# cscott/compressjs

Hardware: AMD Instinct MI355X
Metric: bzip2 -9 compress MB/s on enwik8-shaped input (higher is better)
Workload: dtype u8; 1 GPU; synthetic enwik8-shaped text with phrase reuse calibrated to enwik8's bzip2 -9 ratio (compressjs_amd.synth.enwik_like, seed 2025), 100000000 bytes per GPU, bzip2 -9, 899981-byte blocks; BASELINE.json configs[2]; input_bytes=100000000, compressed_bytes=29488912, blocks_in_flight=128

## Files before the change

### compressjs_amd/csrc/cjs_abi.hip

```cpp
#include "../../include/compressjs_amd.h"
#include "cjs_common.h"
#include "k1_bwt.h"
#include "pipeline.h"
#include "bwtc_host.h"
#include "decode_host.h"
#include <vector>
#include <atomic>
#include <chrono>
#include <thread>
#include <functional>
#include <mutex>
#include <condition_variable>
#include <string.h>
#include <stdlib.h>

static int ensure_device() {
    int n = 0;
    if (hipGetDeviceCount(&n) != hipSuccess || n <= 0) return CJS_E_NOGPU;
    return CJS_OK;
}

static int32_t bwt_batch_impl(const uint8_t* T, const uint32_t* nlen, uint32_t nb, uint32_t cap,
                              uint8_t* U, uint32_t* pidx, int reps, float* ms_out, int linear = 0,
                              int32_t* SAout = nullptr) {
// ... 89 lines not shown
    if (n == 0) return CJS_OK;
    if (!SA) return CJS_E_ARG;
    std::vector<u8> u(n);
    u32 p = 0;
    return bwt_batch_impl(T, &n, 1, n, u.data(), &p, 0, nullptr, 1, SA);
}

extern "C" int32_t cjs_unbwt_linear(const uint8_t* T, uint8_t* U, uint32_t n, uint32_t pidx) {
    if (n == 0) return CJS_OK;
    if (!T || !U || pidx > n) return CJS_E_ARG;
    int rc = ensure_device();
    if (rc) return rc;
    u8 *dT = nullptr, *dU = nullptr; void* ws = nullptr;
    hipStream_t st = nullptr;
    hipError_t e;
    const size_t wsb = (size_t)n * 20 + ((size_t)(n + 4095) / 4096) * 1024 + 256;
#define TRY(x) if ((e = (x)) != hipSuccess) { rc = CJS_E_HIP - (int)e; goto done; }
    TRY(hipStreamCreate(&st));
    TRY(hipMalloc((void**)&dT, n));
    TRY(hipMalloc((void**)&dU, n));
    TRY(hipMalloc(&ws, wsb));
    TRY(hipMemcpyAsync(dT, T, n, hipMemcpyHostToDevice, st));
    TRY(hipMemsetAsync(dU, 0, n, st));
    rc = k6_unbwt_linear(dT, dU, n, pidx, ws, st);
    if (rc) goto done;
    TRY(hipStreamSynchronize(st));
    TRY(hipMemcpy(U, dU, n, hipMemcpyDeviceToHost));
done:
    if (st) (void)hipStreamDestroy(st);
    (void)hipFree(dT); (void)hipFree(dU); (void)hipFree(ws);
    return rc;
#undef TRY
}

extern "C" int32_t cjs_huff_lengths_batch(int64_t* arr, const uint32_t* off, uint32_t count, uint32_t max_len) {
    if (count == 0) return CJS_OK;
    if (!arr || !off || max_len < 1 || max_len > 62) return CJS_E_ARG;
    for (u32 k = 0; k < count; k++) {
        if (off[k + 1] < off[k]) return CJS_E_ARG;
        const u64 len = off[k + 1] - off[k];
        if (len > (1ull << max_len)) return CJS_E_ARG;
    }
    const u32 total = off[count];
    if (total == 0) return CJS_OK;
    int rc = ensure_device();
    if (rc) return rc;
    long long* d_arr = nullptr; u32* d_off = nullptr;
    hipError_t e;
#define TRY(x) if ((e = (x)) != hipSuccess) { rc = CJS_E_HIP - (int)e; goto done; }
    TRY(hipMalloc((void**)&d_arr, (size_t)total * 8));
    TRY(hipMalloc((void**)&d_off, (size_t)(count + 1) * 4));
    TRY(hipMemcpy(d_arr, arr, (size_t)total * 8, hipMemcpyHostToDevice));
    TRY(hipMemcpy(d_off, off, (size_t)(count + 1) * 4, hipMemcpyHostToDevice));
    rc = k3_alloc_lengths_run(d_arr, d_off, count, (int)max_len, nullptr);
    if (rc) goto done;
    TRY(hipDeviceSynchronize());
    TRY(hipMemcpy(arr, d_arr, (size_t)total * 8, hipMemcpyDeviceToHost));
done:
    (void)hipFree(d_arr); (void)hipFree(d_off);
    return rc;
#undef TRY
}
extern "C" int32_t cjs_huff_lengths(int64_t* arr, uint32_t n, uint32_t max_len) {
    const uint32_t off[2] = {0, n};
    return cjs_huff_lengths_batch(arr, off, 1, max_len);
}

extern "C" int32_t cjs_bwt_cyclic(const uint8_t* T, uint8_t* U, uint32_t n, uint32_t* pidx) {
    if (n == 0) { if (pidx) *pidx = 0; return CJS_OK; }
    return cjs_bwt_cyclic_batch(T, &n, 1, n, U, pidx);
}

extern "C" int32_t cjs_dbg_block_stages(const uint8_t* T, const uint32_t* nlen, uint32_t nb, uint32_t cap,
                                        int upto, cjs_dbg_stage_out* o) {
    void* dout = nullptr;
    if (!T || !nlen || !o || nb == 0 || cap == 0 || cap > (1u << 22) - 1) return CJS_E_ARG;
    int rc = ensure_device();
    if (rc) return rc;
    BatchGeom g = make_geom(nb, cap);
    u32 max_n = 0;
    std::vector<u8> text((size_t)nb * g.tstride, 0);
    for (u32 b = 0; b < nb; b++) {
        const u32 n = nlen[b];
        if (n > cap || n == 0) return CJS_E_ARG;
        if (n > max_n) max_n = n;
        u8* dst = text.data() + (size_t)b * g.tstride;
        memcpy(dst, T + (size_t)b * cap, n);
        for (u32 i = 0; i < K1_TPAD; i++) dst[n + i] = dst[i % n];
    }
    void* ws = nullptr;
    hipStream_t st = nullptr;
    hipError_t e;
    Pipe P;
#define TRY(x) if ((e = (x)) != hipSuccess) { rc = CJS_E_HIP - (int)e; goto done; }
    TRY(hipStreamCreate(&st));
    TRY(hipMalloc(&ws, pipe_bytes(g)));
    pipe_carve(P, g, ws);
    TRY(hipMemcpyAsync(P.T, text.data(), text.size(), hipMemcpyHostToDevice, st));
    TRY(hipMemcpyAsync(P.nlen, nlen, nb * 4, hipMemcpyHostToDevice, st));
    TRY(hipMemsetAsync(P.pidx, 0, nb * 4, st));
    if (o->crc_in) { TRY(hipMemcpyAsync(P.crc, o->crc_in, nb * 4, hipMemcpyHostToDevice, st)); }
    else { TRY(hipMemsetAsync(P.crc, 0, nb * 4, st)); }
    if (upto >= 5) {
        P.outCapBytes = ((size_t)nb * ((size_t)cap * 2 + 8192) + 4096 + 255) & ~(size_t)255;
        TRY(hipMalloc(&dout, P.outCapBytes));
        P.out = (u32*)dout;
        rc = k5_stream_begin(P, o->level ? o->level : 9, st);
        if (rc) goto done;
    }
    rc = pipe_run_block_stages(P, max_n, st, upto);
    if (rc) goto done;
    if (upto >= 5) { rc = k5_stream_end(P, st); if (rc) goto done; }
    TRY(hipStreamSynchronize(st));
#define BACK2D(dst, src, rowbytes, srcpitch, dstpitch)                                            \
    if (dst) for (u32 b = 0; b < nb; b++)                                                        \
        TRY(hipMemcpy((char*)(dst) + (size_t)b * (dstpitch), (const char*)(src) + (size_t)b * (srcpitch), \
                      (rowbytes), hipMemcpyDeviceToHost));
    BACK2D(o->U, P.U, max_n, g.stride, cap);
    BACK2D(o->pidx, P.pidx, 4, 4, 4);
    if (upto >= 2) {
        BACK2D(o->A, P.A, ((size_t)max_n + 1) * 2, (size_t)g.stride * 2, ((size_t)cap + 1) * 2);
        BACK2D(o->pos, P.pos, 4, 4, 4);
        BACK2D(o->alpha, P.alpha, 4, 4, 4);
        BACK2D(o->freq, P.freq, 258 * 4, K2_FREQ_PITCH * 4, 258 * 4);
        BACK2D(o->used, P.used, 32, 32, 32);
    }
    if (upto >= 3) {
        BACK2D(o->sel, P.sel, (max_n + 1) / 50 + 2, P.selPitch, (cap + 1) / 50 + 2);
        for (int t = 0; t < 6; t++) {
            BACK2D(o->lens ? o->lens + t * 258 : nullptr, P.lens + t * CJS_LEN_PITCH, 258,
                   CJS_MAX_GROUPS * CJS_LEN_PITCH, 6 * 258);
        }
        BACK2D(o->ngroups, P.ngroups, 4, 4, 4);
        BACK2D(o->nsel, P.nsel, 4, 4, 4);
    }
    if (upto >= 5) {
        BACK2D(o->bitlen, P.bitlen, 8, 8, 8);
        StreamState hs;
        TRY(hipMemcpy(&hs, P.ss, sizeof hs, hipMemcpyDeviceToHost));
        if (hs.overflow) { rc = CJS_E_NOSPACE; goto done; }
        o->stream_bytes = (hs.bits + 7) >> 3;
        if (o->stream && o->stream_cap >= o->stream_bytes) {
            TRY(hipMemcpy(o->stream, P.out, o->stream_bytes, hipMemcpyDeviceToHost));
        }
    }
done:
    if (st) (void)hipStreamDestroy(st);
    (void)hipFree(ws);
    (void)hipFree(dout);
    return rc;
#undef TRY
#undef BACK2D
}

#define CJS_PIN_WORDS 8192u
#define CJS_NSTREAMS 4

struct BwtcBlockJob { u32 len, pidx, nsym, ntri; u32 used[8]; size_t off; bool host; size_t soff; };
struct PinnedU32 {
    u32* p = nullptr; size_t cap = 0;
    int reserve(size_t n) {
        if (n <= cap) return CJS_OK;
        if (p) (void)hipHostFree(p);
        p = nullptr; cap = 0;
        n += n / 8 + 1024;
        const hipError_t e = hipHostMalloc((void**)&p, n * sizeof(u32), hipHostMallocDefault);
        if (e != hipSuccess) { p = nullptr; return CJS_E_HIP - (int)e; }
        cap = n;
        return CJS_OK;
    }
    u32* data() { return p; }
    ~PinnedU32() { if (p) (void)hipHostFree(p); }
// ... 1626 lines not shown
```

### compressjs_amd/csrc/k34_huff.hip

```cpp
#include "pipeline.h"
#include <atomic>

#define HB_PITCH 264
#ifdef K34_TRACE
#define K34_NOW() wall_clock64()
#else
#define K34_NOW() 0ll
#endif
static_assert(HB_PITCH == CJS_LEN_PITCH, "fr2's rows (pipeline.hip) have the pitch of the LDS rows");

template <typename I>
__device__ __forceinline__ int ha_mod(I x, int len) {
    return x < (I)len ? (int)x : x < (I)(2 * len) ? (int)x - len : (int)(x % len);
}

template <typename I>
__device__ int ha_first(const I* a, int len, int i, int nodes_to_move) {
    const int limit = i;
    int k = len - 2;
    while (i >= nodes_to_move && ha_mod(a[i], len) > limit) { k = i; i -= (limit - i + 1); }
    if (i < nodes_to_move - 1) i = nodes_to_move - 1;
    while (k > i + 1) {
        const int t = (i + k) >> 1;
        if (ha_mod(a[t], len) > limit) k = t; else i = t;
    }
    return k;
}

template <typename I>
__device__ void ha_parents(I* a, int len) {
    a[0] += a[1];
    {
        const I none = (I)(~(unsigned long long)0 >> (65 - 8 * sizeof(I)));
        int head = 0, top = 2;
        I vh = a[0];
        I vt = top < len ? a[top] : none;
        for (int tail = 1; tail < len - 1; tail++) {
            I t;
            if (top >= len || vh < vt) { t = vh; a[head++] = tail; vh = head < tail ? a[head] : none; }
            else { t = vt; top++; vt = top < len ? a[top] : none; }
            if (top >= len || (head < tail && vh < vt)) { t += vh; a[head++] = tail + len; vh = head < tail ? a[head] : none; }
            else { t += vt; top++; vt = top < len ? a[top] : none; }
            a[tail] = t;
            if (head == tail) vh = t;
        }
    }
}

template <typename I>
__device__ void ha_depths_serial(I* a, int len, int maxlen) {
    int reloc = len - 2;
    for (int d = 1; d < maxlen - 1 && reloc > 1; d++) reloc = ha_first(a, len, reloc - 1, 0);
    if (ha_mod(a[0], len) >= reloc) {
        int first = len - 2, next = len - 1;
        for (int depth = 1, avail = 2; avail > 0; depth++) {
            const int last = first;
            first = ha_first(a, len, last - 1, 0);
            for (int i = avail - (last - first); i > 0; i--) a[next--] = depth;
            avail = (last - first) << 1;
        }
    } else {
        const int nodes_to_move = reloc;
        int fl = 0;
        for (u32 v = (u32)(reloc - 1); v; v >>= 1) fl++;
        const int insert_depth = maxlen - fl;
        int first = len - 2, next = len - 1;
        int depth = (insert_depth == 1) ? 2 : 1;
        int left = (insert_depth == 1) ? nodes_to_move - 2 : nodes_to_move;
        for (int avail = depth << 1; avail > 0; depth++) {
            const int last = first;
            first = (first <= nodes_to_move) ? first : ha_first(a, len, last - 1, nodes_to_move);
            int offset = 0;
            if (depth >= insert_depth) {
                const int capv = 1 << (depth - insert_depth);
                offset = left < capv ? left : capv;
            } else if (depth == insert_depth - 1) {
                offset = 1;
                if (a[first] == last) first++;
            }
            for (int i = avail - (last - first + offset); i > 0; i--) a[next--] = depth;
            left -= offset;
            avail = (last - first + offset) << 1;
        }
    }
// ... 53 lines not shown
            const int last = first;
            if (first > ntm) {
                int below = 0;
                for (int k0 = 0; k0 < root; k0 += 64) {
                    const int k = k0 + lane;
                    below += (int)__popcll(__ballot(k < root && ha_mod(a[k], len) < last));
                }
                first = below > ntm ? below : ntm;
            }
            int offset = 0;
            if (depth >= insert_depth) {
                const int capv = 1 << (depth - insert_depth);
                offset = left < capv ? left : capv;
            } else if (depth == insert_depth - 1) {
                offset = 1;
                if (a[first] == (I)last) first++;
            }
            const int fill = avail - (last - first + offset);
            if (lane == 0 && fill > 0) cnt[64 + depth] = fill;
            left -= offset;
            avail = (last - first + offset) << 1;
        }
        __builtin_amdgcn_wave_barrier();
        const int f = cnt[64 + lane];
        const int cum = (int)wave_incl_scan_u32((u32)f);
        __builtin_amdgcn_wave_barrier();
        cnt[64 + lane] = cum;
        deep = depth - 2;
    } else {
        const int above = __shfl_up(c, 1);
        const int nl = lane >= 1 ? 2 * above - c : 0;
        cnt[64 + lane] = (int)wave_incl_scan_u32((u32)nl);
    }
    __builtin_amdgcn_wave_barrier();
    for (int j = lane; j < len; j += 64) {
        const int r = len - j;
        int dep = 1;
        for (int D = 1; D <= deep; D++) dep += cnt[64 + D] < r ? 1 : 0;
        a[j] = (I)dep;
    }
    __builtin_amdgcn_wave_barrier();
    return true;
}

__device__ void huff_build_wave(const u32* freq, int S, u8* lens, int* keys, int* arr, int* anc, int* dist, int* cnt, u32* tr = nullptr) {
    const int lane = (int)(threadIdx.x & 63u);
    long long t0_ = tr ? K34_NOW() : 0;
    for (int i = lane; i < S; i += 64) keys[i] = (int)((freq[i] << 9) | (u32)i);
    __builtin_amdgcn_wave_barrier();
    {
        constexpr int M = (CJS_MAX_SYMS + 63) / 64;
        int k[M], r[M];
#pragma unroll
        for (int m = 0; m < M; m++) { const int i = lane + 64 * m; k[m] = i < S ? keys[i] : 0; r[m] = 0; }
        for (int j = 0; j < S; j++) {
            const int kj = keys[j];
#pragma unroll
            for (int m = 0; m < M; m++) r[m] += kj < k[m] ? 1 : 0;
        }
#pragma unroll
        for (int m = 0; m < M; m++) if (lane + 64 * m < S) arr[r[m]] = k[m];
    }
    __builtin_amdgcn_wave_barrier();
    for (int i = lane; i < S; i += 64) keys[i] = arr[i];
    __builtin_amdgcn_wave_barrier();
    for (int i = lane; i < S; i += 64) arr[i] = (int)((u32)keys[i] >> 9);
    __builtin_amdgcn_wave_barrier();
    if (tr && lane == 0) { const long long t1_ = K34_NOW(); atomicAdd(tr, (u32)(t1_ - t0_)); t0_ = t1_; }
    if (lane == 0) ha_parents(arr, S);
    __builtin_amdgcn_wave_barrier();
    if (tr && lane == 0) { const long long t1_ = K34_NOW(); atomicAdd(tr + 1, (u32)(t1_ - t0_)); t0_ = t1_; }
    if (!ha_depths_wave(arr, S, CJS_MAX_BITS, anc, dist, cnt)) {
        if (lane == 0) ha_depths_serial(arr, S, CJS_MAX_BITS);
    }
    if (tr && lane == 0) atomicAdd(tr + 2, (u32)(K34_NOW() - t0_));
    __builtin_amdgcn_wave_barrier();
    for (int i = lane; i < S; i += 64) lens[keys[i] & 0x1FF] = (u8)arr[i];
    __builtin_amdgcn_wave_barrier();
}

#define K34_STAGE_WORDS 1600
#define K34_GROUPS_PER_CHUNK 64
#define K34_PRE ((K34_STAGE_WORDS + 63) / 64)

template <class Body, class Done>
__device__ __forceinline__ void walk_groups(const u16* A, u32 pos, u32 nSel, u32* stage_w, u32 c0, u32 cstep, Body body, Done done) {
    const u32 lane = threadIdx.x & 63u;
    const u32* Aw = (const u32*)A;
    const u32 nchunks = (nSel + K34_GROUPS_PER_CHUNK - 1) / K34_GROUPS_PER_CHUNK;
    u32 pre[K34_PRE];
    auto fetch = [&](u32 c) {
        const u32 sym0 = c * K34_GROUPS_PER_CHUNK * CJS_GROUP;
        const u32 nsym = pos - sym0 < 2u * K34_STAGE_WORDS ? pos - sym0 : 2u * K34_STAGE_WORDS;
        const u32 nwords = (nsym + 1u) >> 1;
#pragma unroll
        for (int k = 0; k < K34_PRE; k++) {
            const u32 j = lane + 64u * (u32)k;
            pre[k] = j < nwords ? Aw[(sym0 >> 1) + j] : 0u;
        }
    };
    if (c0 < nchunks) fetch(c0);
    for (u32 c = c0; c < nchunks; c += cstep) {
        const u32 g0 = c * K34_GROUPS_PER_CHUNK;
#pragma unroll
        for (int k = 0; k < K34_PRE; k++) {
            const u32 j = lane + 64u * (u32)k;
            if (j < K34_STAGE_WORDS) stage_w[j] = pre[k];
        }
        __builtin_amdgcn_wave_barrier();
        if (c + cstep < nchunks) fetch(c + cstep);
        const u32 gi = g0 + lane;
        if (lane < K34_GROUPS_PER_CHUNK && gi < nSel) {
            const u32 cnt = pos - gi * CJS_GROUP < CJS_GROUP ? pos - gi * CJS_GROUP : CJS_GROUP;
            const u32* gw = stage_w + lane * 25u;
            if (cnt == CJS_GROUP) {
                u32 wd[CJS_GROUP / 2];
#pragma unroll
                for (int k = 0; k < CJS_GROUP / 2; k++) wd[k] = gw[k];
#pragma unroll
                for (int k = 0; k < CJS_GROUP / 2; k++) { body(gi, wd[k] & 0xFFFFu); body(gi, wd[k] >> 16); }
            } else {
                for (u32 k = 0; k < cnt; k += 2) {
                    const u32 wd = gw[k >> 1];
                    body(gi, wd & 0xFFFFu);
                    if (k + 1 < cnt) body(gi, wd >> 16);
                }
            }
            done(gi);
        }
        __builtin_amdgcn_wave_barrier();
    }
}

#ifndef K34_SPLIT
#define K34_SPLIT 2
#endif
#define K34_MAX_SEL 18432
#ifdef K34_TRACE
#define K34_T0 long long tprev_ = wall_clock64();
#define K34_STAMP(slot) do { __syncthreads(); if (blockIdx.x == 0 && threadIdx.x == 0) { const long long now_ = wall_clock64(); atomicAdd(&P.k1.stats[K1_STAT_RTRACE + (slot)], (u32)(now_ - tprev_)); tprev_ = now_; } } while (0)
#else
#define K34_T0
#define K34_STAMP(slot) do { } while (0)
#endif

struct K34Blk {
    u32 pos, nSel;
    int S, target;
};
__device__ __forceinline__ K34Blk k34_blk(const Pipe& P, u32 b) {
    K34Blk k;
    k.pos = P.pos[b];
    k.S = (int)P.alpha[b] + 2;
    k.nSel = (k.pos + CJS_GROUP - 1) / CJS_GROUP;
    k.target = k.pos >= 2400 ? 6 : k.pos >= 1200 ? 5 : k.pos >= 600 ? 4 : k.pos >= 200 ? 3 : 2;
    return k;
}

__global__ __launch_bounds__(1024) void k34_assign(Pipe P, u32 it) {
    const BatchGeom g = P.g;
    const u32 b = blockIdx.x / K34_SPLIT, k = blockIdx.x % K34_SPLIT;
    if (P.nlen[b] == 0) return;
    const K34Blk q = k34_blk(P, b);
    const int G = 2 + (int)it, S = q.S;
    if (G > q.target) return;
    const u32 tid = threadIdx.x, w = tid >> 6, lane = tid & 63u;
    const u16* A = P.A + (size_t)b * g.stride;
    u8* sel = P.sel + (size_t)b * P.selPitch;
    u16* cost = P.selCost + (size_t)b * P.selPitch;

    HIP_DYNAMIC_SHARED(u32, pool)
    __shared__ u8 lens[CJS_MAX_GROUPS][HB_PITCH];
    __shared__ u32 fr[CJS_MAX_GROUPS][HB_PITCH];
    __shared__ u64 lens64[HB_PITCH];
    u32* stage_w = pool + w * K34_STAGE_WORDS;
    int (*keys)[HB_PITCH] = (int (*)[HB_PITCH])pool;
    int (*arr)[HB_PITCH] = (int (*)[HB_PITCH])(pool + CJS_MAX_GROUPS * HB_PITCH);
    int (*anc)[HB_PITCH] = (int (*)[HB_PITCH])(pool + 2 * CJS_MAX_GROUPS * HB_PITCH);
    int (*dst)[HB_PITCH] = (int (*)[HB_PITCH])(pool + 3 * CJS_MAX_GROUPS * HB_PITCH);
    int (*dcn)[128] = (int (*)[128])(pool + 4 * CJS_MAX_GROUPS * HB_PITCH);

    u32* rows = P.fr2 + ((size_t)b * 2 + (it & 1u)) * CJS_MAX_GROUPS * HB_PITCH;
    u32* next = P.fr2 + ((size_t)b * 2 + ((it + 1u) & 1u)) * CJS_MAX_GROUPS * HB_PITCH;
    K34_T0
    if (it == 0) {
        const u32* gfreq = P.freq + (size_t)b * K2_FREQ_PITCH;
        for (u32 i = tid; i < (u32)S; i += 1024) { fr[0][i] = gfreq[i]; fr[1][i] = 1; }
    } else {
        for (u32 i = tid; i < (u32)G * HB_PITCH; i += 1024) (&fr[0][0])[i] = rows[i];
    }
    if (k == 0 && G < q.target)
        for (u32 i = tid; i < (u32)(CJS_MAX_GROUPS * HB_PITCH); i += 1024) next[i] = 0;
    __syncthreads();
    K34_STAMP(0);
#ifdef K34_TRACE
    if (w < (u32)G) huff_build_wave(fr[w], S, lens[w], keys[w], arr[w], anc[w], dst[w], dcn[w], blockIdx.x == 0 && w == 0 ? P.k1.stats + K1_STAT_RTRACE + 7 : nullptr);
#else
    if (w < (u32)G) huff_build_wave(fr[w], S, lens[w], keys[w], arr[w], anc[w], dst[w], dcn[w]);
#endif
    __syncthreads();
    K34_STAMP(1);
    for (u32 i = tid; i < (u32)S; i += 1024) {
        u64 v = 0;
        for (int t = 0; t < G; t++) v |= (u64)lens[t][i] << (10 * t);
        lens64[i] = v;
    }
    __syncthreads();
    {
        u64 acc = 0;
        walk_groups(A, q.pos, q.nSel, stage_w, k * 16u + w, 16u * K34_SPLIT,
            [&](u32, u32 sym) { acc += lens64[sym]; },
            [&](u32 gi) {
                u32 best = 0, bc = (u32)(acc & 1023u);
                for (int t = 1; t < G; t++) {
                    const u32 c = (u32)((acc >> (10 * t)) & 1023u);
                    if (c < bc) { best = (u32)t; bc = c; }
                }
                sel[gi] = (u8)best;
                cost[gi] = (u16)bc;
                acc = 0;
            });
    }
    K34_STAMP(2);
    if (G < q.target || k != 0) return;
    if (w < (u32)G) {
        const int l = (int)lane;
        const bool mine = l >= 1 && l <= CJS_MAX_BITS;
        u32 count = 0;
        if (mine) for (int i = 0; i < S; i++) count += lens[w][i] == l ? 1u : 0u;
        u32 c = 0, first = 0; int prev = 0;
        for (int ll = 1; ll <= CJS_MAX_BITS; ll++) {
            const u32 cl = (u32)__shfl((int)count, ll);
            if (!cl) continue;
            c <<= (ll - prev);
            if (ll == l) first = c;
            c += cl;
            prev = ll;
        }
        u32* codes = P.codes + ((size_t)b * CJS_MAX_GROUPS + w) * CJS_LEN_PITCH;
        u8* lout = P.lens + ((size_t)b * CJS_MAX_GROUPS + w) * CJS_LEN_PITCH;
        if (mine && count) for (int i = 0; i < S; i++) if (lens[w][i] == l) codes[i] = first++;
        for (int i = l; i < S; i += 64) lout[i] = lens[w][i];
    }
    if (tid == 0) { P.ngroups[b] = (u32)G; P.nsel[b] = q.nSel; }
    K34_STAMP(3);
}

__global__ __launch_bounds__(1024) void k34_split(Pipe P, u32 it) {
    const BatchGeom g = P.g;
    const u32 b = blockIdx.x / K34_SPLIT, k = blockIdx.x % K34_SPLIT;
    if (P.nlen[b] == 0) return;
    const K34Blk q = k34_blk(P, b);
    const int G = 2 + (int)it;
    if (G >= q.target) return;
    const u32 tid = threadIdx.x, w = tid >> 6;
    const u32 nSel = q.nSel;
    const u16* A = P.A + (size_t)b * g.stride;
    const u8* sel = P.sel + (size_t)b * P.selPitch;
    const u16* cost = P.selCost + (size_t)b * P.selPitch;

    HIP_DYNAMIC_SHARED(u32, pool)
    __shared__ u32 fr[CJS_MAX_GROUPS][HB_PITCH];
    __shared__ u32 chist[1024];
    __shared__ u32 cnt[8];
    __shared__ u32 scan_sh[20];
    __shared__ u32 s_which, s_cstar, s_keep;
    __shared__ __attribute__((aligned(16))) u8 selL[K34_MAX_SEL];
    u32* stage_w = pool + w * K34_STAGE_WORDS;
    K34_T0
    u16* costL = (u16*)pool;
    for (u32 i = tid; i < (nSel + 3u) >> 2; i += 1024) ((u32*)selL)[i] = ((const u32*)sel)[i];
    for (u32 i = tid; i < (nSel + 1u) >> 1; i += 1024) ((u32*)costL)[i] = ((const u32*)cost)[i];
    if (tid < 8) cnt[tid] = 0;
    chist[tid] = 0;
    for (u32 i = tid; i < (u32)(CJS_MAX_GROUPS * HB_PITCH); i += 1024) (&fr[0][0])[i] = 0;
    __syncthreads();
    for (u32 g0 = 0; g0 < nSel; g0 += 1024) {
        const u32 gi = g0 + tid;
        const u32 v = gi < nSel ? selL[gi] : 0xFFu;
        for (int t = 0; t < G; t++) {
            const u64 m = __ballot(v == (u32)t);
            if ((tid & 63u) == 0 && m) atomicAdd(&cnt[t], (u32)__popcll(m));
        }
    }
    __syncthreads();
    if (tid == 0) {
        u32 wh = 0;
        for (int t = 1; t < G; t++) if (cnt[t] > cnt[wh]) wh = (u32)t;
        s_which = wh;
    }
    __syncthreads();
    const u32 which = s_which;
    for (u32 gi = tid; gi < nSel; gi += 1024)
        if (selL[gi] == which) atomicAdd(&chist[costL[gi]], 1u);
    __syncthreads();
    {
        const u32 half = cnt[which] >> 1;
        u32 tot;
        const u32 mine = chist[tid];
        const u32 lower = block_excl_scan_1024(mine, scan_sh, &tot);
        if (lower <= half && half < lower + mine) { s_cstar = tid; s_keep = half - lower; }
    }
    __syncthreads();
    {
        const u32 cstar = s_cstar, keep = s_keep;
        const u32 chunk = (nSel + 1023u) / 1024u;
        const u32 lo = tid * chunk < nSel ? tid * chunk : nSel;
        const u32 hi = lo + chunk < nSel ? lo + chunk : nSel;
        u32 eq = 0;
        for (u32 gi = lo; gi < hi; gi++) eq += (selL[gi] == which && costL[gi] == cstar) ? 1u : 0u;
        u32 total;
        u32 rank = block_excl_scan_1024(eq, scan_sh, &total);
        for (u32 gi = lo; gi < hi; gi++) {
            u32 v = selL[gi];
            if (v == which) {
                const u32 c = costL[gi];
                if (c > cstar) v = (u32)G;
                else if (c == cstar) { if (rank >= keep) v = (u32)G; rank++; }
            }
            selL[gi] = (u8)v;
        }
    }
    __syncthreads();
    K34_STAMP(4);
    {
        u64 hot = 0;
        walk_groups(A, q.pos, nSel, stage_w, k * 16u + w, 16u * K34_SPLIT,
            [&](u32 gi, u32 sym) {
                if (sym < 8u) hot += 1ull << (8u * sym);
                else atomicAdd(&fr[selL[gi]][sym], 1u);
            },
            [&](u32 gi) {
                u32* row = fr[selL[gi]];
#pragma unroll
                for (u32 sy = 0; sy < 8u; sy++) {
                    const u32 c = (u32)(hot >> (8u * sy)) & 255u;
                    if (c) atomicAdd(&row[sy], c);
                }
                hot = 0;
            });
    }
    __syncthreads();
    K34_STAMP(5);
    u32* next = P.fr2 + ((size_t)b * 2 + ((it + 1u) & 1u)) * CJS_MAX_GROUPS * HB_PITCH;
    for (u32 i = tid; i < (u32)(CJS_MAX_GROUPS * HB_PITCH); i += 1024) {
        const u32 v = (&fr[0][0])[i];
        if (v) atomicAdd(&next[i], v);
    }
    K34_STAMP(6);
}

int k34_run(Pipe P, hipStream_t stream) {
    const size_t dyn = (size_t)16 * K34_STAGE_WORDS * 4;
    static std::atomic<unsigned> lds_set[64];
    int dev = 0;
    HIP_CHECK_RET(hipGetDevice(&dev));
    if (dev < 0 || dev >= 64 || !lds_set[dev].load(std::memory_order_acquire)) {
        HIP_CHECK_RET(hipFuncSetAttribute((const void*)k34_assign, hipFuncAttributeMaxDynamicSharedMemorySize, (int)(16 * K34_STAGE_WORDS * 4)));
        HIP_CHECK_RET(hipFuncSetAttribute((const void*)k34_split, hipFuncAttributeMaxDynamicSharedMemorySize, (int)(16 * K34_STAGE_WORDS * 4)));
        if (dev >= 0 && dev < 64) lds_set[dev].store(1u, std::memory_order_release);
    }
    if (P.selPitch > K34_MAX_SEL) return CJS_E_ARG;
    for (u32 it = 0; it + 2u <= CJS_MAX_GROUPS; it++) {
        hipLaunchKernelGGL(k34_assign, dim3(P.g.nb * K34_SPLIT), dim3(1024), dyn, stream, P, it);
        if (it + 3u <= CJS_MAX_GROUPS) hipLaunchKernelGGL(k34_split, dim3(P.g.nb * K34_SPLIT), dim3(1024), dyn, stream, P, it);
    }
    HIP_CHECK_RET(hipGetLastError());
#ifdef K34_TRACE
    {
        u32 h[10];
        HIP_CHECK_RET(hipMemcpyAsync(h, P.k1.stats + K1_STAT_RTRACE, sizeof h, hipMemcpyDeviceToHost, stream));
        HIP_CHECK_RET(hipStreamSynchronize(stream));
        fprintf(stderr, "k34 trace (us, block 0 / workgroup 0, summed over iterations): assign load %.1f build %.1f lens64+walk %.1f codes %.1f | split count/median/move %.1f recount %.1f flush %.1f | table 0: sort %.1f parents %.1f depths %.1f\n",
                h[0] / 100.0, h[1] / 100.0, h[2] / 100.0, h[3] / 100.0, h[4] / 100.0, h[5] / 100.0, h[6] / 100.0, h[7] / 100.0, h[8] / 100.0, h[9] / 100.0);
    }
#endif
    return CJS_OK;
}

#define K3_WAVE_MAX 2048
__global__ __launch_bounds__(64) void k3_alloc_lengths(long long* arr, const u32* off, u32 count, int maxlen) {
    const u32 t = blockIdx.x;
    if (t >= count) return;
    __shared__ int anc[K3_WAVE_MAX], dist[K3_WAVE_MAX], cnt[128];
    long long* a = arr + off[t];
    const int len = (int)(off[t + 1] - off[t]);
    const bool one = threadIdx.x == 0;
    if (len == 2) { if (one) { a[0] = 1; a[1] = 1; } }
    else if (len == 1) { if (one) a[0] = 1; }
    else if (len > K3_WAVE_MAX || maxlen > HA_DCAP - 1) { if (one) ha_allocate<long long>(a, len, maxlen); }
    else if (len > 2) {
        if (one) ha_parents<long long>(a, len);
        __syncthreads();
        if (!ha_depths_wave<long long>(a, len, maxlen, anc, dist, cnt)) {
            if (one) ha_depths_serial<long long>(a, len, maxlen);
        }
    }
}
int k3_alloc_lengths_run(long long* d_arr, const u32* d_off, u32 count, int maxlen, hipStream_t stream) {
    hipLaunchKernelGGL(k3_alloc_lengths, dim3(count), dim3(64), 0, stream, d_arr, d_off, count, maxlen);
    HIP_CHECK_RET(hipGetLastError());
    return CJS_OK;
}
```

### compressjs_amd/csrc/pipeline.h

```cpp
#pragma once
#include "cjs_common.h"
#include "devutil.h"
#include "k1_bwt.h"

#define K2_SEG 1024
#define K2_FREQ_PITCH 260
#define CJS_MAX_SYMS 258
#define CJS_MAX_GROUPS 6
#define CJS_GROUP 50
#define CJS_MAX_BITS 20
#define CJS_LEN_PITCH 264

#define K5_NONE (-0x40000000)
#define K5_TGROUPS 80u
#define K5_TILE (K5_TGROUPS * CJS_GROUP)
#define K5_TILES(g) ((g).stride / K5_TILE + 2u)
#define K5_HDR_WORDS 6144

struct StreamState {
    u64 bits;
    u32 crc;
    u32 overflow;
};

struct Pipe {
    BatchGeom g;
    u32 segs;
    u8* T;
    u32* nlen;
    u32* crc;
    K1Buf k1;
    u8* U;
    u32* pidx;
    u32* used;
    u32* alpha;
    u32* nruns;
    u32* tileCnt;
    u32* symCnt;
    u8* RHsym;
    u32* RHpos;
    int* Ltab;
    u8* J;
    u16* A;
    u32* pos;
    u32* freq;
    u8* sel;
    u32 selPitch;
    u8* lens;
    u32* codes;
    u32* ngroups;
    u32* nsel;
    u16* selCost;
    u32* fr2;
    u32* hdr;
    u32* hbits;
    u32* tileBits;
    u64* bitlen;
    u64* bitoff;
    StreamState* ss;
    u32* out;
    u64 outCapBytes;
    u64* snap;
};

struct K0Buf {
    const u8* in;
    u64 in_len;
    u64 ntiles;
    u64 nchunks;
    u32 maxBlocks;
    u64* tileA;
    u64* tileB;
    u64* tileC;
    u64* chunk;
    u64* blkStart;
    u64* blkEnd;
    u64* blkAdj;
    u64* blkRe;
    u32* blkN;
    u32* nBlocks;
    u64* specEnd;
    u64* specC;
    u64* specBad;
};
size_t k0_bytes(u64 in_len, u32 cap);
void k0_carve(K0Buf& K, const u8* d_in, u64 in_len, u32 cap, void* ws);
int k0_prepass(K0Buf K, u32 cap, hipStream_t stream);
#define K0_PHASE_FAIL 0xFFFFFFFFu
int k0_scans(K0Buf K, hipStream_t stream);
int k0_eval(K0Buf K, u64 pos, hipStream_t stream);
int k0_phase_plan(K0Buf K, u32 cap, u64 t0, u64 own_len, u32 last, u64 total, hipStream_t stream);

int k6_unbwt_linear(const u8* dT, u8* dU, u32 n, u32 pidx, void* ws, hipStream_t stream);
int k2_run(Pipe P, u32 max_n, hipStream_t stream);
int k10_model_run(Pipe P, u32* sylt, u32* tot, u32* ntri, u32 ostride, u32 ocap, hipStream_t stream);
int k34_run(Pipe P, hipStream_t stream);
int k3_alloc_lengths_run(long long* d_arr, const u32* d_off, u32 count, int maxlen, hipStream_t stream);
int k5_run(Pipe P, u32 max_n, hipStream_t stream, hipEvent_t after = nullptr, hipEvent_t done = nullptr, hipEvent_t crc_ready = nullptr);
int k5_stream_begin(Pipe P, int level, hipStream_t stream, bool zero = true);
int k5_stream_end(Pipe P, hipStream_t stream);
int k5_shift_bits_run(const u8* d_in, u64 nbytes, u32 s, u8* d_out, hipStream_t stream);
int k0_batch(K0Buf K, Pipe P, u32 first_block, u32 cap, hipStream_t stream, u32 crc_parts, hipStream_t side = nullptr, hipEvent_t ev_pad = nullptr, hipEvent_t ev_crc = nullptr);
size_t pipe_bytes(const BatchGeom& g);
void pipe_carve(Pipe& P, const BatchGeom& g, void* base);
int pipe_run_block_stages(Pipe& P, u32 max_n, hipStream_t stream, int upto, hipEvent_t after = nullptr,
                          hipEvent_t done = nullptr);
```

### compressjs_amd/csrc/pipeline.hip

```cpp
#include "pipeline.h"
#include <string.h>

static inline size_t al256(size_t x) { return (x + 255) & ~(size_t)255; }

size_t pipe_bytes(const BatchGeom& g) {
    size_t tot = 0;
    tot += al256((size_t)g.nb * g.tstride);
    tot += al256((size_t)g.nb * g.stride);
    tot += al256((size_t)g.nb * (g.stride + 1) * 4);
    tot += 2 * al256((size_t)g.nb * g.stride);
    tot += al256((size_t)g.nb * (g.stride / K2_SEG) * 256 * 4);
    tot += al256((size_t)g.nb * g.stride * 2);
    tot += 2 * al256((size_t)g.nb * g.rtiles * 4);
    tot += 16 * al256((size_t)g.nb * 8 * 4);
    tot += al256((size_t)g.nb * K2_FREQ_PITCH * 4);
    const u32 selPitch = (g.stride / CJS_GROUP + 64) & ~63u;
    tot += al256((size_t)g.nb * selPitch);
    tot += al256((size_t)g.nb * CJS_MAX_GROUPS * CJS_LEN_PITCH);
    tot += al256((size_t)g.nb * CJS_MAX_GROUPS * CJS_LEN_PITCH * 4);
    tot += al256((size_t)g.nb * selPitch * 2);
    tot += al256((size_t)g.nb * 2 * CJS_MAX_GROUPS * CJS_LEN_PITCH * 4);
    tot += al256((size_t)g.nb * K5_HDR_WORDS * 4);
    tot += al256((size_t)g.nb * K5_TILES(g) * 4);
    tot += 4 * al256((size_t)g.nb * 8);
    tot += k1_workspace_bytes(g);
    return tot;
}

void pipe_carve(Pipe& P, const BatchGeom& g, void* base) {
    memset(&P, 0, sizeof P);
    P.g = g;
    P.segs = g.stride / K2_SEG;
    char* p = (char*)base;
#define TAKE(field, type, bytes) P.field = (type)p; p += al256(bytes)
    TAKE(T, u8*, (size_t)g.nb * g.tstride);
    TAKE(U, u8*, (size_t)g.nb * g.stride);
    TAKE(RHpos, u32*, (size_t)g.nb * (g.stride + 1) * 4);
    TAKE(RHsym, u8*, (size_t)g.nb * g.stride);
    TAKE(J, u8*, (size_t)g.nb * g.stride);
    TAKE(Ltab, int*, (size_t)g.nb * P.segs * 256 * 4);
    TAKE(A, u16*, (size_t)g.nb * g.stride * 2);
    TAKE(tileCnt, u32*, (size_t)g.nb * g.rtiles * 4);
    TAKE(symCnt, u32*, (size_t)g.nb * g.rtiles * 4);
    TAKE(nlen, u32*, (size_t)g.nb * 4);
    TAKE(crc, u32*, (size_t)g.nb * 4);
    TAKE(pidx, u32*, (size_t)g.nb * 4);
    TAKE(used, u32*, (size_t)g.nb * 8 * 4);
    TAKE(alpha, u32*, (size_t)g.nb * 4);
    TAKE(nruns, u32*, (size_t)g.nb * 4);
    TAKE(pos, u32*, (size_t)g.nb * 4);
    TAKE(ngroups, u32*, (size_t)g.nb * 4);
    TAKE(nsel, u32*, (size_t)g.nb * 4);
    TAKE(bitlen, u64*, (size_t)g.nb * 8);
    TAKE(bitoff, u64*, (size_t)(g.nb + 1) * 8);
    TAKE(freq, u32*, (size_t)g.nb * K2_FREQ_PITCH * 4);
    P.selPitch = (g.stride / CJS_GROUP + 64) & ~63u;
    TAKE(sel, u8*, (size_t)g.nb * P.selPitch);
    TAKE(lens, u8*, (size_t)g.nb * CJS_MAX_GROUPS * CJS_LEN_PITCH);
    TAKE(codes, u32*, (size_t)g.nb * CJS_MAX_GROUPS * CJS_LEN_PITCH * 4);
    TAKE(selCost, u16*, (size_t)g.nb * P.selPitch * 2);
    TAKE(fr2, u32*, (size_t)g.nb * 2 * CJS_MAX_GROUPS * CJS_LEN_PITCH * 4);
    TAKE(hdr, u32*, (size_t)g.nb * K5_HDR_WORDS * 4);
    TAKE(tileBits, u32*, (size_t)g.nb * K5_TILES(g) * 4);
    TAKE(hbits, u32*, (size_t)g.nb * 4);
    TAKE(ss, StreamState*, sizeof(StreamState));
#undef TAKE
    p = (char*)(((uintptr_t)p + 255) & ~(uintptr_t)255);
    k1_carve(P.k1, g, p);
    P.k1.T = P.T;
    P.k1.nlen = P.nlen;
    P.k1.U = P.U;
    P.k1.pidx = P.pidx;
}

int pipe_run_block_stages(Pipe& P, u32 max_n, hipStream_t stream, int upto, hipEvent_t after, hipEvent_t done) {
    int rc = k1_run(P.k1, P.g, max_n, stream);
    if (rc || upto <= 1) return rc;
    rc = k2_run(P, max_n, stream);
    if (rc || upto <= 2) return rc;
    rc = k34_run(P, stream);
    if (rc || upto <= 4) return rc;
    return k5_run(P, max_n, stream, after, done);
}
```

Before: 15700 MB/s.

## Split k34 table refinement into tables/cost/median/recount kernels with wide grids

Restructures each Huffman-table refinement iteration from two per-block 1024-thread kernels (two workgroups per block) into four kernels. Table building runs once per block and writes lens64 to global memory. The group-cost walk and the frequency recount run as 2D grids with many small 256-thread workgroups per block, and per-table group counts are accumulated atomically during the cost pass, so the median kernel no longer needs its own counting pass. The aim is to spread the group walks across far more CUs than before and drop the dynamic-LDS setup; in exchange it adds kernel launches, global round-trips for lens64 and sel, and more global atomics. It also lets the debug-stage entry point skip zero-length blocks instead of rejecting them.

```diff
diff --git a/compressjs_amd/csrc/cjs_abi.hip b/compressjs_amd/csrc/cjs_abi.hip
--- a/compressjs_amd/csrc/cjs_abi.hip
+++ b/compressjs_amd/csrc/cjs_abi.hip
@@ -195,12 +195,14 @@
     std::vector<u8> text((size_t)nb * g.tstride, 0);
     for (u32 b = 0; b < nb; b++) {
         const u32 n = nlen[b];
-        if (n > cap || n == 0) return CJS_E_ARG;
+        if (n > cap) return CJS_E_ARG;
+        if (n == 0) continue;
         if (n > max_n) max_n = n;
         u8* dst = text.data() + (size_t)b * g.tstride;
         memcpy(dst, T + (size_t)b * cap, n);
         for (u32 i = 0; i < K1_TPAD; i++) dst[n + i] = dst[i % n];
     }
+    if (max_n == 0) return CJS_E_ARG;
     void* ws = nullptr;
     hipStream_t st = nullptr;
     hipError_t e;
diff --git a/compressjs_amd/csrc/k34_huff.hip b/compressjs_amd/csrc/k34_huff.hip
--- a/compressjs_amd/csrc/k34_huff.hip
+++ b/compressjs_amd/csrc/k34_huff.hip
@@ -1,5 +1,4 @@
 #include "pipeline.h"
-#include <atomic>
 
 #define HB_PITCH 264
 #ifdef K34_TRACE
@@ -219,12 +218,19 @@
 #define K34_STAGE_WORDS 1600
 #define K34_GROUPS_PER_CHUNK 64
 #define K34_PRE ((K34_STAGE_WORDS + 63) / 64)
-
-template <class Body, class Done>
-__device__ __forceinline__ void walk_groups(const u16* A, u32 pos, u32 nSel, u32* stage_w, u32 c0, u32 cstep, Body body, Done done) {
+#define K34_WALK_WAVES 4
+#ifndef K34_CPW
+#define K34_CPW 4
+#endif
+#define K34_WG_CHUNKS (K34_WALK_WAVES * K34_CPW)
+static_assert(K34_GROUPS_PER_CHUNK * K34_CPW < 1024, "k34_cost sums a wave's per-table group counts in 10-bit fields");
+
+template <class Begin, class Body, class Done>
+__device__ __forceinline__ void walk_groups(const u16* A, u32 pos, u32 nSel, u32* stage_w, u32 c0, u32 cstep, u32 cend, Begin begin, Body body, Done done) {
     const u32 lane = threadIdx.x & 63u;
     const u32* Aw = (const u32*)A;
-    const u32 nchunks = (nSel + K34_GROUPS_PER_CHUNK - 1) / K34_GROUPS_PER_CHUNK;
+    const u32 nall = (nSel + K34_GROUPS_PER_CHUNK - 1) / K34_GROUPS_PER_CHUNK;
+    const u32 nchunks = nall < cend ? nall : cend;
     u32 pre[K34_PRE];
     auto fetch = [&](u32 c) {
         const u32 sym0 = c * K34_GROUPS_PER_CHUNK * CJS_GROUP;
@@ -250,6 +256,7 @@
         if (lane < K34_GROUPS_PER_CHUNK && gi < nSel) {
             const u32 cnt = pos - gi * CJS_GROUP < CJS_GROUP ? pos - gi * CJS_GROUP : CJS_GROUP;
             const u32* gw = stage_w + lane * 25u;
+            begin(gi);
             if (cnt == CJS_GROUP) {
                 u32 wd[CJS_GROUP / 2];
 #pragma unroll
@@ -269,15 +276,12 @@
     }
 }
 
-#ifndef K34_SPLIT
-#define K34_SPLIT 2
-#endif
 #define K34_MAX_SEL 18432
 #ifdef K34_TRACE
-#define K34_T0 long long tprev_ = wall_clock64();
-#define K34_STAMP(slot) do { __syncthreads(); if (blockIdx.x == 0 && threadIdx.x == 0) { const long long now_ = wall_clock64(); atomicAdd(&P.k1.stats[K1_STAT_RTRACE + (slot)], (u32)(now_ - tprev_)); tprev_ = now_; } } while (0)
+#define K34_T0(pred) const bool traced_ = (pred); long long tprev_ = wall_clock64();
+#define K34_STAMP(slot) do { __syncthreads(); if (traced_ && threadIdx.x == 0) { const long long now_ = wall_clock64(); atomicAdd(&P.k1.stats[K1_STAT_RTRACE + (slot)], (u32)(now_ - tprev_)); tprev_ = now_; } } while (0)
 #else
-#define K34_T0
+#define K34_T0(pred)
 #define K34_STAMP(slot) do { } while (0)
 #endif
 
@@ -294,72 +298,50 @@
     return k;
 }
 
-__global__ __launch_bounds__(1024) void k34_assign(Pipe P, u32 it) {
-    const BatchGeom g = P.g;
-    const u32 b = blockIdx.x / K34_SPLIT, k = blockIdx.x % K34_SPLIT;
+__global__ __launch_bounds__(512) void k34_tables(Pipe P, u32 it) {
+    const u32 b = blockIdx.x;
     if (P.nlen[b] == 0) return;
     const K34Blk q = k34_blk(P, b);
     const int G = 2 + (int)it, S = q.S;
     if (G > q.target) return;
     const u32 tid = threadIdx.x, w = tid >> 6, lane = tid & 63u;
-    const u16* A = P.A + (size_t)b * g.stride;
-    u8* sel = P.sel + (size_t)b * P.selPitch;
-    u16* cost = P.selCost + (size_t)b * P.selPitch;
-
-    HIP_DYNAMIC_SHARED(u32, pool)
+
     __shared__ u8 lens[CJS_MAX_GROUPS][HB_PITCH];
     __shared__ u32 fr[CJS_MAX_GROUPS][HB_PITCH];
-    __shared__ u64 lens64[HB_PITCH];
-    u32* stage_w = pool + w * K34_STAGE_WORDS;
-    int (*keys)[HB_PITCH] = (int (*)[HB_PITCH])pool;
-    int (*arr)[HB_PITCH] = (int (*)[HB_PITCH])(pool + CJS_MAX_GROUPS * HB_PITCH);
-    int (*anc)[HB_PITCH] = (int (*)[HB_PITCH])(pool + 2 * CJS_MAX_GROUPS * HB_PITCH);
-    int (*dst)[HB_PITCH] = (int (*)[HB_PITCH])(pool + 3 * CJS_MAX_GROUPS * HB_PITCH);
-    int (*dcn)[128] = (int (*)[128])(pool + 4 * CJS_MAX_GROUPS * HB_PITCH);
+    __shared__ int keys[CJS_MAX_GROUPS][HB_PITCH], arr[CJS_MAX_GROUPS][HB_PITCH];
+    __shared__ int anc[CJS_MAX_GROUPS][HB_PITCH], dst[CJS_MAX_GROUPS][HB_PITCH];
+    __shared__ int dcn[CJS_MAX_GROUPS][128];
 
     u32* rows = P.fr2 + ((size_t)b * 2 + (it & 1u)) * CJS_MAX_GROUPS * HB_PITCH;
     u32* next = P.fr2 + ((size_t)b * 2 + ((it + 1u) & 1u)) * CJS_MAX_GROUPS * HB_PITCH;
-    K34_T0
+    K34_T0(b == 0)
     if (it == 0) {
         const u32* gfreq = P.freq + (size_t)b * K2_FREQ_PITCH;
-        for (u32 i = tid; i < (u32)S; i += 1024) { fr[0][i] = gfreq[i]; fr[1][i] = 1; }
+        for (u32 i = tid; i < (u32)S; i += 512) { fr[0][i] = gfreq[i]; fr[1][i] = 1; }
     } else {
-        for (u32 i = tid; i < (u32)G * HB_PITCH; i += 1024) (&fr[0][0])[i] = rows[i];
-    }
-    if (k == 0 && G < q.target)
-        for (u32 i = tid; i < (u32)(CJS_MAX_GROUPS * HB_PITCH); i += 1024) next[i] = 0;
+        for (u32 i = tid; i < (u32)G * HB_PITCH; i += 512) (&fr[0][0])[i] = rows[i];
+    }
+    if (G < q.target) {
+        for (u32 i = tid; i < (u32)(CJS_MAX_GROUPS * HB_PITCH); i += 512) next[i] = 0;
+        if (tid < 8) P.tabCnt[(size_t)b * 8 + tid] = 0;
+    }
     __syncthreads();
     K34_STAMP(0);
 #ifdef K34_TRACE
-    if (w < (u32)G) huff_build_wave(fr[w], S, lens[w], keys[w], arr[w], anc[w], dst[w], dcn[w], blockIdx.x == 0 && w == 0 ? P.k1.stats + K1_STAT_RTRACE + 7 : nullptr);
+    if (w < (u32)G) huff_build_wave(fr[w], S, lens[w], keys[w], arr[w], anc[w], dst[w], dcn[w], b == 0 && w == 0 ? P.k1.stats + K1_STAT_RTRACE + 9 : nullptr);
 #else
     if (w < (u32)G) huff_build_wave(fr[w], S, lens[w], keys[w], arr[w], anc[w], dst[w], dcn[w]);
 #endif
     __syncthreads();
     K34_STAMP(1);
-    for (u32 i = tid; i < (u32)S; i += 1024) {
+    u64* l64 = P.lens64 + (size_t)b * HB_PITCH;
+    for (u32 i = tid; i < (u32)S; i += 512) {
         u64 v = 0;
         for (int t = 0; t < G; t++) v |= (u64)lens[t][i] << (10 * t);
-        lens64[i] = v;
-    }
-    __syncthreads();
-    {
-        u64 acc = 0;
-        walk_groups(A, q.pos, q.nSel, stage_w, k * 16u + w, 16u * K34_SPLIT,
-            [&](u32, u32 sym) { acc += lens64[sym]; },
-            [&](u32 gi) {
-                u32 best = 0, bc = (u32)(acc & 1023u);
-                for (int t = 1; t < G; t++) {
-                    const u32 c = (u32)((acc >> (10 * t)) & 1023u);
-                    if (c < bc) { best = (u32)t; bc = c; }
-                }
-                sel[gi] = (u8)best;
-                cost[gi] = (u16)bc;
-                acc = 0;
-            });
+        l64[i] = v;
     }
     K34_STAMP(2);
-    if (G < q.target || k != 0) return;
+    if (G < q.target) return;
     if (w < (u32)G) {
         const int l = (int)lane;
         const bool mine = l >= 1 && l <= CJS_MAX_BITS;
@@ -383,56 +365,88 @@
     K34_STAMP(3);
 }
 
-__global__ __launch_bounds__(1024) void k34_split(Pipe P, u32 it) {
+__global__ __launch_bounds__(64 * K34_WALK_WAVES) void k34_cost(Pipe P, u32 it) {
     const BatchGeom g = P.g;
-    const u32 b = blockIdx.x / K34_SPLIT, k = blockIdx.x % K34_SPLIT;
+    const u32 b = blockIdx.y;
+    if (P.nlen[b] == 0) return;
+    const K34Blk q = k34_blk(P, b);
+    const int G = 2 + (int)it, S = q.S;
+    if (G > q.target) return;
+    const u32 cbase = blockIdx.x * K34_WG_CHUNKS;
+    if (cbase * K34_GROUPS_PER_CHUNK >= q.nSel) return;
+    const u32 tid = threadIdx.x, w = tid >> 6, lane = tid & 63u;
+    const u16* A = P.A + (size_t)b * g.stride;
+    u8* sel = P.sel + (size_t)b * P.selPitch;
+    u16* cost = P.selCost + (size_t)b * P.selPitch;
+
+    __shared__ u64 lens64[HB_PITCH];
+    __shared__ u32 stage[K34_WALK_WAVES][K34_STAGE_WORDS];
+    __shared__ u32 wcnt[8];
+    K34_T0(b == 0 && blockIdx.x == 0)
+    const u64* l64 = P.lens64 + (size_t)b * HB_PITCH;
+    for (u32 i = tid; i < (u32)S; i += 64 * K34_WALK_WAVES) lens64[i] = l64[i];
+    if (tid < 8) wcnt[tid] = 0;
+    __syncthreads();
+    K34_STAMP(4);
+    u64 acc = 0, mine = 0;
+    walk_groups(A, q.pos, q.nSel, stage[w], cbase + w, K34_WALK_WAVES, cbase + K34_WG_CHUNKS,
+        [&](u32) { },
+        [&](u32, u32 sym) { acc += lens64[sym]; },
+        [&](u32 gi) {
+            u32 best = 0, bc = (u32)(acc & 1023u);
+            for (int t = 1; t < G; t++) {
+                const u32 c = (u32)((acc >> (10 * t)) & 1023u);
+                if (c < bc) { best = (u32)t; bc = c; }
+            }
+            sel[gi] = (u8)best;
+            cost[gi] = (u16)bc;
+            mine += 1ull << (10u * best);
+            acc = 0;
+        });
+    if (G < q.target) {
+        for (int m = 32; m; m >>= 1) mine += __shfl_xor(mine, m);
+        if (lane < (u32)G) {
+            const u32 c = (u32)(mine >> (10u * lane)) & 1023u;
+            if (c) atomicAdd(&wcnt[lane], c);
+        }
+        __syncthreads();
+        if (tid < (u32)G && wcnt[tid]) atomicAdd(&P.tabCnt[(size_t)b * 8 + tid], wcnt[tid]);
+    }
+    K34_STAMP(5);
+}
+
+__global__ __launch_bounds__(1024) void k34_median(Pipe P, u32 it) {
+    const u32 b = blockIdx.x;
     if (P.nlen[b] == 0) return;
     const K34Blk q = k34_blk(P, b);
     const int G = 2 + (int)it;
     if (G >= q.target) return;
-    const u32 tid = threadIdx.x, w = tid >> 6;
+    const u32 tid = threadIdx.x;
     const u32 nSel = q.nSel;
-    const u16* A = P.A + (size_t)b * g.stride;
-    const u8* sel = P.sel + (size_t)b * P.selPitch;
+    u8* sel = P.sel + (size_t)b * P.selPitch;
     const u16* cost = P.selCost + (size_t)b * P.selPitch;
 
-    HIP_DYNAMIC_SHARED(u32, pool)
-    __shared__ u32 fr[CJS_MAX_GROUPS][HB_PITCH];
     __shared__ u32 chist[1024];
-    __shared__ u32 cnt[8];
     __shared__ u32 scan_sh[20];
-    __shared__ u32 s_which, s_cstar, s_keep;
+    __shared__ u32 s_cstar, s_keep;
     __shared__ __attribute__((aligned(16))) u8 selL[K34_MAX_SEL];
-    u32* stage_w = pool + w * K34_STAGE_WORDS;
-    K34_T0
-    u16* costL = (u16*)pool;
+    __shared__ __attribute__((aligned(16))) u16 costL[K34_MAX_SEL];
+    K34_T0(b == 0)
     for (u32 i = tid; i < (nSel + 3u) >> 2; i += 1024) ((u32*)selL)[i] = ((const u32*)sel)[i];
     for (u32 i = tid; i < (nSel + 1u) >> 1; i += 1024) ((u32*)costL)[i] = ((const u32*)cost)[i];
-    if (tid < 8) cnt[tid] = 0;
     chist[tid] = 0;
-    for (u32 i = tid; i < (u32)(CJS_MAX_GROUPS * HB_PITCH); i += 1024) (&fr[0][0])[i] = 0;
-    __syncthreads();
-    for (u32 g0 = 0; g0 < nSel; g0 += 1024) {
-        const u32 gi = g0 + tid;
-        const u32 v = gi < nSel ? selL[gi] : 0xFFu;
-        for (int t = 0; t < G; t++) {
-            const u64 m = __ballot(v == (u32)t);
-            if ((tid & 63u) == 0 && m) atomicAdd(&cnt[t], (u32)__popcll(m));
-        }
-    }
-    __syncthreads();
-    if (tid == 0) {
-        u32 wh = 0;
-        for (int t = 1; t < G; t++) if (cnt[t] > cnt[wh]) wh = (u32)t;
-        s_which = wh;
-    }
-    __syncthreads();
-    const u32 which = s_which;
+    u32 which = 0, most;
+    {
+        const u32* cnt = P.tabCnt + (size_t)b * 8;
+        most = cnt[0];
+        for (int t = 1; t < G; t++) { const u32 c = cnt[t]; if (c > most) { which = (u32)t; most = c; } }
+    }
+    __syncthreads();
     for (u32 gi = tid; gi < nSel; gi += 1024)
         if (selL[gi] == which) atomicAdd(&chist[costL[gi]], 1u);
     __syncthreads();
     {
-        const u32 half = cnt[which] >> 1;
+        const u32 half = most >> 1;
         u32 tot;
         const u32 mine = chist[tid];
         const u32 lower = block_excl_scan_1024(mine, scan_sh, &tot);
@@ -459,16 +473,39 @@
         }
     }
     __syncthreads();
-    K34_STAMP(4);
+    for (u32 i = tid; i < (nSel + 3u) >> 2; i += 1024) ((u32*)sel)[i] = ((const u32*)selL)[i];
+    K34_STAMP(6);
+}
+
+__global__ __launch_bounds__(64 * K34_WALK_WAVES) void k34_recount(Pipe P, u32 it) {
+    const BatchGeom g = P.g;
+    const u32 b = blockIdx.y;
+    if (P.nlen[b] == 0) return;
+    const K34Blk q = k34_blk(P, b);
+    const int G = 2 + (int)it;
+    if (G >= q.target) return;
+    const u32 cbase = blockIdx.x * K34_WG_CHUNKS;
+    if (cbase * K34_GROUPS_PER_CHUNK >= q.nSel) return;
+    const u32 tid = threadIdx.x, w = tid >> 6;
+    const u16* A = P.A + (size_t)b * g.stride;
+    const u8* sel = P.sel + (size_t)b * P.selPitch;
+
+    __shared__ u32 fr[CJS_MAX_GROUPS][HB_PITCH];
+    __shared__ u32 stage[K34_WALK_WAVES][K34_STAGE_WORDS];
+    K34_T0(b == 0 && blockIdx.x == 0)
+    const u32 cells = (u32)(G + 1) * HB_PITCH;
+    for (u32 i = tid; i < cells; i += 64 * K34_WALK_WAVES) (&fr[0][0])[i] = 0;
+    __syncthreads();
     {
         u64 hot = 0;
-        walk_groups(A, q.pos, nSel, stage_w, k * 16u + w, 16u * K34_SPLIT,
-            [&](u32 gi, u32 sym) {
+        u32* row = fr[0];
+        walk_groups(A, q.pos, q.nSel, stage[w], cbase + w, K34_WALK_WAVES, cbase + K34_WG_CHUNKS,
+            [&](u32 gi) { row = fr[sel[gi]]; },
+            [&](u32, u32 sym) {
                 if (sym < 8u) hot += 1ull << (8u * sym);
-                else atomicAdd(&fr[selL[gi]][sym], 1u);
+                else atomicAdd(&row[sym], 1u);
             },
-            [&](u32 gi) {
-                u32* row = fr[selL[gi]];
+            [&](u32) {
 #pragma unroll
                 for (u32 sy = 0; sy < 8u; sy++) {
                     const u32 c = (u32)(hot >> (8u * sy)) & 255u;
@@ -478,38 +515,35 @@
             });
     }
     __syncthreads();
-    K34_STAMP(5);
+    K34_STAMP(7);
     u32* next = P.fr2 + ((size_t)b * 2 + ((it + 1u) & 1u)) * CJS_MAX_GROUPS * HB_PITCH;
-    for (u32 i = tid; i < (u32)(CJS_MAX_GROUPS * HB_PITCH); i += 1024) {
+    for (u32 i = tid; i < cells; i += 64 * K34_WALK_WAVES) {
         const u32 v = (&fr[0][0])[i];
         if (v) atomicAdd(&next[i], v);
     }
-    K34_STAMP(6);
+    K34_STAMP(8);
 }
 
 int k34_run(Pipe P, hipStream_t stream) {
-    const size_t dyn = (size_t)16 * K34_STAGE_WORDS * 4;
-    static std::atomic<unsigned> lds_set[64];
-    int dev = 0;
-    HIP_CHECK_RET(hipGetDevice(&dev));
-    if (dev < 0 || dev >= 64 || !lds_set[dev].load(std::memory_order_acquire)) {
-        HIP_CHECK_RET(hipFuncSetAttribute((const void*)k34_assign, hipFuncAttributeMaxDynamicSharedMemorySize, (int)(16 * K34_STAGE_WORDS * 4)));
-        HIP_CHECK_RET(hipFuncSetAttribute((const void*)k34_split, hipFuncAttributeMaxDynamicSharedMemorySize, (int)(16 * K34_STAGE_WORDS * 4)));
-        if (dev >= 0 && dev < 64) lds_set[dev].store(1u, std::memory_order_release);
-    }
     if (P.selPitch > K34_MAX_SEL) return CJS_E_ARG;
+    const u32 chunks = (P.selPitch + K34_GROUPS_PER_CHUNK - 1) / K34_GROUPS_PER_CHUNK;
+    const dim3 wide((chunks + K34_WG_CHUNKS - 1) / K34_WG_CHUNKS, P.g.nb);
     for (u32 it = 0; it + 2u <= CJS_MAX_GROUPS; it++) {
-        hipLaunchKernelGGL(k34_assign, dim3(P.g.nb * K34_SPLIT), dim3(1024), dyn, stream, P, it);
-        if (it + 3u <= CJS_MAX_GROUPS) hipLaunchKernelGGL(k34_split, dim3(P.g.nb * K34_SPLIT), dim3(1024), dyn, stream, P, it);
+        hipLaunchKernelGGL(k34_tables, dim3(P.g.nb), dim3(512), 0, stream, P, it);
+        hipLaunchKernelGGL(k34_cost, wide, dim3(64 * K34_WALK_WAVES), 0, stream, P, it);
+        if (it + 3u <= CJS_MAX_GROUPS) {
+            hipLaunchKernelGGL(k34_median, dim3(P.g.nb), dim3(1024), 0, stream, P, it);
+            hipLaunchKernelGGL(k34_recount, wide, dim3(64 * K34_WALK_WAVES), 0, stream, P, it);
+        }
     }
     HIP_CHECK_RET(hipGetLastError());
 #ifdef K34_TRACE
     {
-        u32 h[10];
+        u32 h[12];
         HIP_CHECK_RET(hipMemcpyAsync(h, P.k1.stats + K1_STAT_RTRACE, sizeof h, hipMemcpyDeviceToHost, stream));
         HIP_CHECK_RET(hipStreamSynchronize(stream));
-        fprintf(stderr, "k34 trace (us, block 0 / workgroup 0, summed over iterations): assign load %.1f build %.1f lens64+walk %.1f codes %.1f | split count/median/move %.1f recount %.1f flush %.1f | table 0: sort %.1f parents %.1f depths %.1f\n",
-                h[0] / 100.0, h[1] / 100.0, h[2] / 100.0, h[3] / 100.0, h[4] / 100.0, h[5] / 100.0, h[6] / 100.0, h[7] / 100.0, h[8] / 100.0, h[9] / 100.0);
+        fprintf(stderr, "k34 trace (us, block 0 / its first workgroup, summed over iterations): tables load %.1f build %.1f lens64 %.1f codes %.1f | cost load %.1f walk+counts %.1f | median/move %.1f | recount zero+walk %.1f flush %.1f | table 0: sort %.1f parents %.1f depths %.1f\n",
+                h[0] / 100.0, h[1] / 100.0, h[2] / 100.0, h[3] / 100.0, h[4] / 100.0, h[5] / 100.0, h[6] / 100.0, h[7] / 100.0, h[8] / 100.0, h[9] / 100.0, h[10] / 100.0, h[11] / 100.0);
     }
 #endif
     return CJS_OK;
diff --git a/compressjs_amd/csrc/pipeline.h b/compressjs_amd/csrc/pipeline.h
--- a/compressjs_amd/csrc/pipeline.h
+++ b/compressjs_amd/csrc/pipeline.h
@@ -52,6 +52,8 @@
     u32* nsel;
     u16* selCost;
     u32* fr2;
+    u64* lens64;
+    u32* tabCnt;
     u32* hdr;
     u32* hbits;
     u32* tileBits;
diff --git a/compressjs_amd/csrc/pipeline.hip b/compressjs_amd/csrc/pipeline.hip
--- a/compressjs_amd/csrc/pipeline.hip
+++ b/compressjs_amd/csrc/pipeline.hip
@@ -20,6 +20,8 @@
     tot += al256((size_t)g.nb * CJS_MAX_GROUPS * CJS_LEN_PITCH * 4);
     tot += al256((size_t)g.nb * selPitch * 2);
     tot += al256((size_t)g.nb * 2 * CJS_MAX_GROUPS * CJS_LEN_PITCH * 4);
+    tot += al256((size_t)g.nb * CJS_LEN_PITCH * 8);
+    tot += al256((size_t)g.nb * 8 * 4);
     tot += al256((size_t)g.nb * K5_HDR_WORDS * 4);
     tot += al256((size_t)g.nb * K5_TILES(g) * 4);
     tot += 4 * al256((size_t)g.nb * 8);
@@ -60,6 +62,8 @@
     TAKE(codes, u32*, (size_t)g.nb * CJS_MAX_GROUPS * CJS_LEN_PITCH * 4);
     TAKE(selCost, u16*, (size_t)g.nb * P.selPitch * 2);
     TAKE(fr2, u32*, (size_t)g.nb * 2 * CJS_MAX_GROUPS * CJS_LEN_PITCH * 4);
+    TAKE(lens64, u64*, (size_t)g.nb * CJS_LEN_PITCH * 8);
+    TAKE(tabCnt, u32*, (size_t)g.nb * 8 * 4);
     TAKE(hdr, u32*, (size_t)g.nb * K5_HDR_WORDS * 4);
     TAKE(tileBits, u32*, (size_t)g.nb * K5_TILES(g) * 4);
     TAKE(hbits, u32*, (size_t)g.nb * 4);
```

Result: no change. 15760 MB/s, median of 6 (+0.4%).
